# codename0og/codename-rvc-fork-3

Hardware: AMD Instinct MI355X
Metric: 48 kHz audio samples/sec end-to-end VC (higher is better)
Workload: dtype f32 (vocoder ResBlock convs and upsamplers, HuBERT, RMVPE's U-Net convs: fp32 operands as exact bf16x3 splits on the bf16 matrix cores -- six products of order <= 2^-16 per multiply-add, fp32 accumulate; everything else fp32 / fp64)

## Files before the change

### codename-rvc-fork-3_amd/csrc/linbf.hip

```cpp
#include <stdlib.h>

#include <mutex>
#include <vector>

#include "conv.h"

namespace rvc {

struct LinBfParams {
    const void *a = nullptr;
    const void *xs = nullptr;
    const float *bias = nullptr;
    float *y = nullptr;
    void *ys = nullptr;
    int M = 0, K = 0;
    int64_t N = 0, n_pad = 0;
    int mode = 0;
    int64_t x_row_stride = 0, x_plane = 0;
    int steps_per_part = 0;
    int n_col_blocks = 0;
};

constexpr int LBF_BN = 128, LBF_NTH = 512;
constexpr int LBF_SLAB_STEP = 12 * 1024;
constexpr int LBF_B_CHUNK = 3 * LBF_BN * 64;
typedef void __attribute__((address_space(3))) *lbf_lptr_t;

template <int MI>
struct LbfGeom {
    static constexpr int BM = 64 * MI;
    static constexpr int A_STEP = 2 * MI * 3 * 1024;
    static constexpr int D = MI == 2 ? 2 : 1;
    static constexpr int A_RING = 2 * (D + 1), B_RING = D + 1;
    static constexpr int NPIECE = 2 * 2 * MI * 3 + 24;
    static constexpr int UPW = (NPIECE + 7) / 8;
    static constexpr int LDS_USED = A_RING * A_STEP + B_RING * LBF_B_CHUNK;
    static_assert(LDS_USED <= 163840, "");
};

template <int MI>
__global__ void __launch_bounds__(LBF_NTH) __attribute__((amdgpu_waves_per_eu(2, 2)))
linbf_kernel(const LinBfParams p) {
    using GM = LbfGeom<MI>;
    constexpr int BM = GM::BM, A_STEP = GM::A_STEP, D = GM::D, A_RING = GM::A_RING, B_RING = GM::B_RING, NPIECE = GM::NPIECE, UPW = GM::UPW;
    extern __shared__ __attribute__((aligned(16))) unsigned char lbf_smem[];
    unsigned char *const a_ring = lbf_smem;
    unsigned char *const b_ring = lbf_smem + A_RING * A_STEP;
    const int tid = threadIdx.x, lane = tid & 63;
    const int wave = __builtin_amdgcn_readfirstlane(tid >> 6);
    __builtin_assume(wave >= 0 && wave < 8);
    const int wm = wave >> 2, wn = wave & 3;
    const int half = lane >> 5, l31 = lane & 31;
    const int n_m = p.M / BM;
    const int xcd = blockIdx.x & 7, slot = blockIdx.x >> 3;
// ... 98 lines not shown
                    if (p.bias) o += *reinterpret_cast<const f32x4 *>(p.bias + mb + 4 * half + 8 * (2 * rp + g));
#pragma unroll
                    for (int r = 0; r < 4; ++r) o[r] = 0.5f * o[r] * (1.f + erff(o[r] * 0.70710678118654752f));
                    v[g][0] = f32x2{o[0], o[1]};
                    v[g][1] = f32x2{o[2], o[3]};
                }
#pragma unroll
                for (int sp = 0; sp < 3; ++sp) {
                    unsigned w[2][2];
#pragma unroll
                    for (int g = 0; g < 2; ++g)
#pragma unroll
                        for (int h = 0; h < 2; ++h) {
                            w[g][h] = split_word(v[g][h]);
                            v[g][h] = split_rest(v[g][h], w[g][h]);
                        }
                    const unsigned s0 = half ? w[0][0] : w[1][0], s1 = half ? w[0][1] : w[1][1];
                    const unsigned r0 = (unsigned)__shfl_xor((int)s0, 32, 64), r1 = (unsigned)__shfl_xor((int)s1, 32, 64);
                    const u32x4 out = half ? u32x4{r0, r1, w[1][0], w[1][1]} : u32x4{w[0][0], w[0][1], r0, r1};
                    const int m = mb + 16 * rp + 8 * half;
                    if (live) *reinterpret_cast<u32x4 *>(reinterpret_cast<unsigned char *>(p.ys) + (((int64_t)sp * p.n_pad + n) * p.M + m) * 2) = out;
                }
            }
        }
        return;
    }
#pragma unroll
    for (int mi = 0; mi < MI; ++mi) {
        const int64_t n = n0 + nrow;
        if (n >= p.N) continue;
        const int mb = m0 + wm * 32 * MI + mi * 32 + 4 * half;
#pragma unroll
        for (int rg = 0; rg < 4; ++rg) {
            const int m = mb + 8 * rg;
            f32x4 o;
#pragma unroll
            for (int r = 0; r < 4; ++r) o[r] = acc[mi][4 * rg + r];
            if (p.mode == 2) {
                *reinterpret_cast<f32x4 *>(p.y + ((int64_t)part * p.N + n) * p.M + m) = o;
                continue;
            }
            if (p.bias) o += *reinterpret_cast<const f32x4 *>(p.bias + m);
            if (p.mode == 0) {
                *reinterpret_cast<f32x4 *>(p.y + n * p.M + m) = o;
                continue;
            }
#pragma unroll
            for (int r = 0; r < 4; ++r) o[r] = 0.5f * o[r] * (1.f + erff(o[r] * 0.70710678118654752f));
            *reinterpret_cast<f32x4 *>(p.y + n * p.M + m) = o;
        }
    }
}

__global__ void __launch_bounds__(256) split_rows_kernel(const float *__restrict__ x, unsigned char *__restrict__ xs, int64_t n_rows,
                                                          int64_t n_pad, int k) {
    const int64_t i4 = (int64_t)blockIdx.x * 256 + threadIdx.x;
    const int64_t total4 = n_rows * k / 4;
    if (i4 >= total4) return;
    const f32x4 v = *reinterpret_cast<const f32x4 *>(x + i4 * 4);
    f32x2 v0 = {v.x, v.y}, v1 = {v.z, v.w};
#pragma unroll
    for (int sp = 0; sp < 3; ++sp) {
        const unsigned w0 = split_word(v0), w1 = split_word(v1);
        *reinterpret_cast<u32x2 *>(xs + ((int64_t)sp * n_pad * k + i4 * 4) * 2) = u32x2{w0, w1};
        v0 = split_rest(v0, w0);
        v1 = split_rest(v1, w1);
    }
}

__device__ __forceinline__ float ln_row_mean(float sum, float inv_m) {
    float mean = sum * inv_m;
    asm volatile("" : "+v"(mean));
    return mean;
}

template <int PER_LANE>
__global__ void __launch_bounds__(256) ln_reduce_kernel(const float *__restrict__ parts, int n_parts, const float *__restrict__ bias,
                                                         const float *__restrict__ res, const float *__restrict__ gamma,
                                                         const float *__restrict__ beta, float eps, float *__restrict__ y,
                                                         unsigned char *__restrict__ ys, int64_t n_rows, int64_t n_pad) {
    constexpr int M = 64 * PER_LANE, Q = PER_LANE / 4;
    const int lane = threadIdx.x & 63;
    const int64_t n = (int64_t)blockIdx.x * 4 + (threadIdx.x >> 6);
    if (n >= n_rows) return;
    f32x4 v[Q];
#pragma unroll
    for (int q = 0; q < Q; ++q) {
        const int m = (q * 64 + lane) * 4;
        f32x4 a = bias ? *reinterpret_cast<const f32x4 *>(bias + m) : f32x4{0.f, 0.f, 0.f, 0.f};
        for (int s = 0; s < n_parts; ++s) a += *reinterpret_cast<const f32x4 *>(parts + ((int64_t)s * n_rows + n) * M + m);
        if (res) a += *reinterpret_cast<const f32x4 *>(res + n * M + m);
        v[q] = a;
    }
    float sum = 0.f;
#pragma unroll
    for (int q = 0; q < Q; ++q) sum += (v[q].x + v[q].y) + (v[q].z + v[q].w);
#pragma unroll
    for (int o = 32; o > 0; o >>= 1) sum += __shfl_xor(sum, o, 64);
    const float mean = ln_row_mean(sum, 1.f / M);
    float sq = 0.f;
#pragma unroll
    for (int q = 0; q < Q; ++q) {
        const f32x4 d = v[q] - mean;
        sq += (d.x * d.x + d.y * d.y) + (d.z * d.z + d.w * d.w);
    }
#pragma unroll
    for (int o = 32; o > 0; o >>= 1) sq += __shfl_xor(sq, o, 64);
    const float rstd = 1.f / sqrtf(sq * (1.f / M) + eps);
#pragma unroll
    for (int q = 0; q < Q; ++q) {
        const int m = (q * 64 + lane) * 4;
        f32x4 o = (v[q] - mean) * rstd;
        if (gamma) o *= *reinterpret_cast<const f32x4 *>(gamma + m);
        if (beta) o += *reinterpret_cast<const f32x4 *>(beta + m);
        if (y) *reinterpret_cast<f32x4 *>(y + n * M + m) = o;
        if (ys) {
            f32x2 v0 = {o.x, o.y}, v1 = {o.z, o.w};
#pragma unroll
            for (int sp = 0; sp < 3; ++sp) {
                const unsigned w0 = split_word(v0), w1 = split_word(v1);
                *reinterpret_cast<u32x2 *>(ys + (((int64_t)sp * n_pad + n) * M + m) * 2) = u32x2{w0, w1};
                v0 = split_rest(v0, w0);
                v1 = split_rest(v1, w1);
            }
        }
    }
}

template <int MI>
static int linbf_launch(LinBfParams p, int parts, hipStream_t stream) {
    if (reserve_whole_cu((const void *)linbf_kernel<MI>, "linear bf16x3 (pre-split)")) return 1;
    p.n_col_blocks = (int)ceil_div(p.N, LBF_BN);
    const int n_m = p.M / LbfGeom<MI>::BM;
    dim3 grid((unsigned)(ceil_div((int64_t)p.n_col_blocks * n_m, 8) * 8), (unsigned)parts, 1);
    hipLaunchKernelGGL(linbf_kernel<MI>, grid, dim3(LBF_NTH), LDS_WHOLE_CU, stream, p);
    RVC_LAUNCH_CHECK();
    return 0;
}

}

using namespace rvc;

extern "C" int rvc_split_rows_bf16x3(const float *x_dev, void *xs_dev, int64_t n_rows, int64_t n_rows_padded, int k, void *stream) {
    if (!x_dev || !xs_dev) return fail("rvc_split_rows_bf16x3: null pointer");
    if (k % 16 || n_rows_padded < n_rows || n_rows < 0) return fail("rvc_split_rows_bf16x3: k must be a multiple of 16, n_rows_padded >= n_rows");
    if (n_rows == 0) return 0;
    const int64_t total4 = n_rows * k / 4;
    hipLaunchKernelGGL(split_rows_kernel, dim3((unsigned)ceil_div(total4, 256)), dim3(256), 0, (hipStream_t)stream, x_dev,
                       reinterpret_cast<unsigned char *>(xs_dev), n_rows, n_rows_padded, k);
    RVC_LAUNCH_CHECK();
    return 0;
}

namespace {
int linbf_dispatch(const char *who, const void *xs_dev, int64_t x_row_stride, int64_t x_plane, const void *a_dev, const float *bias_dev,
                   float *y_dev, void *ys_dev, int64_t n_rows, int64_t n_rows_padded, int in_features, int out_features, int mode,
                   int k_parts, void *stream) {
    if (!xs_dev || !a_dev) return fail("%s: null pointer", who);
    if (out_features % 128 || in_features % 16) return fail("%s: out_features must be a multiple of 128, in_features of 16", who);
    if (mode < 0 || mode > 3) return fail("%s: mode must be 0 (fp32 + bias), 1 (bias + GELU -> planes), 2 (partial sums) or 3 (bias + GELU -> fp32)", who);
    if ((mode == 1) ? !ys_dev : !y_dev) return fail("%s: the output of mode %d is missing", who, mode);
    if (k_parts < 1 || (in_features / 32) % k_parts || in_features % 32) return fail("%s: in_features must be a multiple of 32 and k_parts divide in_features / 32", who);
    if (k_parts > 1 && mode != 2) return fail("%s: several K parts only produce partial sums (mode 2)", who);
    if (n_rows_padded % LBF_BN || n_rows_padded < n_rows) return fail("%s: n_rows_padded must be a multiple of 128 and >= n_rows", who);
    if (!fits_2gib((int64_t)out_features * in_features, 6) || !fits_2gib(3 * x_plane, 2) ||
        !fits_2gib((n_rows_padded + LBF_BN) * x_row_stride, 2))
        return fail("%s: an operand exceeds 2 GiB", who);
    if (x_row_stride % 8) return fail("%s: rows must start on 16-byte boundaries", who);
    if (n_rows <= 0) return 0;
    LinBfParams p;
    p.a = a_dev; p.xs = xs_dev; p.bias = bias_dev; p.y = y_dev; p.ys = ys_dev;
    p.M = out_features; p.K = in_features; p.N = n_rows; p.n_pad = n_rows_padded; p.mode = mode;
    p.x_row_stride = x_row_stride; p.x_plane = x_plane;
    p.steps_per_part = in_features / 16 / k_parts;
    const int64_t cols = ceil_div(n_rows, LBF_BN);
    const int cus = 256;
    auto cost = [&](int rows_per_block, double rel) {
        if (out_features % rows_per_block) return 1e30;
        return (double)ceil_div(cols * (out_features / rows_per_block) * k_parts, cus) * rel;
    };
    static const int by_cu_time = knob("RVC_LBF_TP", 0);
    if (by_cu_time) {
        auto cu_time = [&](int rows_per_block, double rel) { return out_features % rows_per_block ? 1e30 : cols * (out_features / rows_per_block) * k_parts * rel; };
        const double t128 = cu_time(128, 1.0), t192 = cu_time(192, 1.5 * 0.85), t256 = cu_time(256, 1.85);
        if (t192 <= t128 && t192 <= t256) return linbf_launch<3>(p, k_parts, (hipStream_t)stream);
        if (t256 < t128) return linbf_launch<4>(p, k_parts, (hipStream_t)stream);
        return linbf_launch<2>(p, k_parts, (hipStream_t)stream);
    }
    const double c128 = cost(128, 1.0), c192 = cost(192, 1.5 * 0.85), c256 = cost(256, 1.85);
    if (c256 < c128 && c256 <= c192) return linbf_launch<4>(p, k_parts, (hipStream_t)stream);
    const bool use192 = c192 < c128;
    return use192 ? linbf_launch<3>(p, k_parts, (hipStream_t)stream) : linbf_launch<2>(p, k_parts, (hipStream_t)stream);
}
}

extern "C" int rvc_linear_bf16x3_presplit(const void *xs_dev, const void *a_dev, const float *bias_dev, float *y_dev, void *ys_dev,
                                          int64_t n_rows, int64_t n_rows_padded, int in_features, int out_features, int mode, int k_parts,
                                          void *stream) {
    return linbf_dispatch("rvc_linear_bf16x3_presplit", xs_dev, in_features, n_rows_padded * in_features, a_dev, bias_dev, y_dev, ys_dev,
                          n_rows, n_rows_padded, in_features, out_features, mode, k_parts, stream);
}

extern "C" int rvc_conv1d_frames_bf16x3(const void *xs_dev, int64_t n_frames_in, int64_t n_frames_in_padded, int channels, int taps,
                                        int stride, const void *a_dev, const float *bias_dev, float *y_dev, void *ys_dev,
                                        int64_t n_frames_out_padded, int out_channels, int mode, void *stream) {
    if (taps < 1 || stride < 1 || channels < 8 || n_frames_in_padded < n_frames_in) return fail("rvc_conv1d_frames_bf16x3: bad argument");
    if (mode == 2) return fail("rvc_conv1d_frames_bf16x3: modes 0 (fp32 + bias), 1 (bias + GELU -> planes), 3 (bias + GELU -> fp32)");
    const int64_t n_out = n_frames_in >= taps ? (n_frames_in - taps) / stride + 1 : 0;
    return linbf_dispatch("rvc_conv1d_frames_bf16x3", xs_dev, (int64_t)stride * channels, n_frames_in_padded * channels, a_dev, bias_dev,
                          y_dev, ys_dev, n_out, n_frames_out_padded, taps * channels, out_channels, mode, 1, stream);
}

extern "C" int rvc_bias_residual_layernorm_bf16x3(const float *parts_dev, int n_parts, const float *bias_dev, const float *res_dev,
                                                  const float *gamma_dev, const float *beta_dev, float eps, float *y_dev, void *ys_dev,
                                                  int64_t n_rows, int64_t n_rows_padded, int features, void *stream) {
    if (!parts_dev || (!y_dev && !ys_dev)) return fail("rvc_bias_residual_layernorm_bf16x3: null pointer");
    if (n_parts < 1 || n_rows_padded < n_rows) return fail("rvc_bias_residual_layernorm_bf16x3: bad argument");
    if (n_rows <= 0) return 0;
    dim3 grid((unsigned)ceil_div(n_rows, 4));
    unsigned char *ys = reinterpret_cast<unsigned char *>(ys_dev);
    hipStream_t st = (hipStream_t)stream;
    if (features == 768)
        hipLaunchKernelGGL(ln_reduce_kernel<12>, grid, dim3(256), 0, st, parts_dev, n_parts, bias_dev, res_dev, gamma_dev, beta_dev, eps, y_dev, ys, n_rows, n_rows_padded);
    else if (features == 1024)
        hipLaunchKernelGGL(ln_reduce_kernel<16>, grid, dim3(256), 0, st, parts_dev, n_parts, bias_dev, res_dev, gamma_dev, beta_dev, eps, y_dev, ys, n_rows, n_rows_padded);
    else if (features == 256)
        hipLaunchKernelGGL(ln_reduce_kernel<4>, grid, dim3(256), 0, st, parts_dev, n_parts, bias_dev, res_dev, gamma_dev, beta_dev, eps, y_dev, ys, n_rows, n_rows_padded);
    else
        return fail("rvc_bias_residual_layernorm_bf16x3: features must be 256, 768 or 1024 (HuBERT-base: 768)");
    RVC_LAUNCH_CHECK();
    return 0;
}
```

### codename-rvc-fork-3_amd/rvc_amd/_native.py

```python
from __future__ import annotations

import ctypes
import threading
import os
from ctypes import POINTER, c_char_p, c_float, c_int, c_int64, c_size_t, c_void_p

import torch

_HERE = os.path.dirname(os.path.abspath(__file__))
LIB_PATH = os.path.join(_HERE, "_lib", "librvc_amd.so")
if os.environ.get("RVC_AMD_LIB"):
    LIB_PATH = os.path.abspath(os.environ["RVC_AMD_LIB"])
    print(f"[rvc_amd] RVC_AMD_LIB: loading {LIB_PATH} instead of the product library", flush=True)


class NativeError(RuntimeError):
    pass


if not os.path.isfile(LIB_PATH):
    raise ImportError(
        f"{LIB_PATH} is missing: build it with `python -c 'import __graft_entry__ as g; g.build()'` "
        "(hipcc --offload-arch=gfx950).  rvc_amd has no fallback path without its HIP library.")

# ... 62 lines not shown
    "rvc_decoder_set_tap": (c_int, [c_void_p, c_int, c_void_p]),
    "rvc_decoder_set_concurrency_hint": (c_int, [c_void_p, c_int]),
    "rvc_decoder_set_branch_parallel": (c_int, [c_void_p, c_int]),
    "rvc_posconv_bf16x3_weight_bytes": (c_int, [c_int, c_int, c_int, POINTER(c_size_t)]),
    "rvc_posconv_bf16x3_pack_weight": (c_int, [c_void_p, c_int, c_int, c_int, c_void_p, c_void_p]),
    "rvc_posconv_gelu_bf16x3": (c_int, [c_void_p, c_void_p, c_void_p, c_void_p, c_int64, c_int, c_int, c_int, c_int, c_void_p]),
    "rvc_hubert_conv0_workspace_bytes": (c_int, [c_int, POINTER(c_size_t)]),
    "rvc_hubert_conv0_frames_bf16x3": (c_int, [c_void_p, c_int64, c_void_p, c_int, c_int, c_int, c_void_p, c_void_p, c_float, c_void_p,
                                               c_size_t, c_void_p, c_int64, c_void_p]),
    "rvc_conv1d_frames_bf16x3": (c_int, [c_void_p, c_int64, c_int64, c_int, c_int, c_int, c_void_p, c_void_p, c_void_p, c_void_p, c_int64,
                                         c_int, c_int, c_void_p]),
    "rvc_conv1d_pack_weight": (c_int, [c_void_p, c_int, c_int, c_int, c_void_p, c_void_p]),
    "rvc_conv1d_forward": (c_int, [c_void_p, c_void_p, c_void_p, c_void_p, c_void_p, c_void_p, c_int, c_int, c_int,
                                   c_int64, c_int, c_int, c_float, c_float, c_void_p]),
    "rvc_conv1d_wino_pack_weight": (c_int, [c_void_p, c_int, c_int, c_int, c_void_p, c_void_p]),
    "rvc_conv1d_wino_forward": (c_int, [c_void_p, c_void_p, c_void_p, c_void_p, c_void_p, c_void_p, c_int, c_int, c_int,
                                        c_int64, c_int, c_int, c_float, c_float, c_void_p]),
    "rvc_conv1d_winobf_weight_bytes": (c_int, [c_int, c_int, c_int, POINTER(c_size_t)]),
    "rvc_conv1d_winobf_pack_weight": (c_int, [c_void_p, c_int, c_int, c_int, c_void_p, c_void_p]),
    "rvc_conv1d_winobf_forward": (c_int, [c_void_p, c_void_p, c_void_p, c_void_p, c_void_p, c_void_p, c_int, c_int, c_int,
                                          c_int64, c_int, c_int, c_float, c_float, c_void_p]),
    "rvc_resblock_bf16x3_weight_bytes": (c_int, [c_int, c_int, POINTER(c_size_t)]),
    "rvc_resblock_bf16x3_pack_weight": (c_int, [c_void_p, c_void_p, c_int, c_int, c_void_p, c_void_p]),
    "rvc_resblock_bf16x3_forward": (c_int, [c_void_p, c_void_p, c_void_p, c_void_p, c_void_p, c_void_p, c_int, c_int, c_int64, c_int,
                                            c_int, c_float, c_float, c_void_p]),
    "rvc_resblock_bf16w_weight_bytes": (c_int, [c_int, c_int, POINTER(c_size_t)]),
    "rvc_resblock_bf16w_pack_weight": (c_int, [c_void_p, c_void_p, c_int, c_int, c_void_p, c_void_p]),
    "rvc_resblock_bf16w_forward": (c_int, [c_void_p, c_void_p, c_void_p, c_void_p, c_void_p, c_void_p, c_int, c_int, c_int64, c_int,
                                           c_int, c_float, c_float, c_void_p]),
    "rvc_resblock_bf16x3_set_enabled": (c_int, [c_int]),
    "rvc_upsample_bf16x3_weight_bytes": (c_int, [c_int, c_int, c_int, c_int, c_int, c_int, POINTER(c_size_t)]),
    "rvc_upsample_bf16x3_pack_weight": (c_int, [c_void_p, c_void_p, c_void_p, c_int, c_int, c_int, c_int, c_int, c_int, c_void_p, c_void_p]),
    "rvc_upsample_bf16x3_forward": (c_int, [c_void_p, c_void_p, c_int64, c_void_p, c_void_p, c_void_p, c_int, c_int, c_int, c_int64, c_int, c_int,
                                            c_int, c_int, c_int, c_int, c_float, c_void_p]),
    "rvc_conv1d_f16x2_weight_bytes": (c_int, [c_int, c_int, POINTER(c_size_t)]),
    "rvc_conv1d_f16x2_pack_weight": (c_int, [c_void_p, c_int, c_int, c_void_p, c_void_p]),
    "rvc_conv1d_f16x2_forward": (c_int, [c_void_p, c_void_p, c_void_p, c_void_p, c_void_p, c_void_p, c_int, c_int, c_int64, c_int,
                                         c_int, c_float, c_float, c_void_p]),
    "rvc_decoder_set_arithmetic": (c_int, [c_void_p, c_int]),
    "rvc_conv1d_bf16w_weight_bytes": (c_int, [c_int, c_int, POINTER(c_size_t)]),
    "rvc_conv1d_bf16w_pack_weight": (c_int, [c_void_p, c_int, c_int, c_void_p, c_void_p]),
    "rvc_conv1d_bf16w_forward": (c_int, [c_void_p, c_void_p, c_void_p, c_void_p, c_void_p, c_void_p, c_int, c_int, c_int64, c_int,
                                         c_int, c_float, c_float, c_void_p]),
    "rvc_gemm_bf16x3_weight_bytes": (c_int, [c_int, c_int, POINTER(c_size_t)]),
    "rvc_gemm_bf16x3_pack_weight": (c_int, [c_void_p, c_int, c_int, c_int, c_void_p, c_void_p]),
    "rvc_linear_bf16x3": (c_int, [c_void_p, c_void_p, c_void_p, c_void_p, c_void_p, c_int64, c_int, c_int, c_int, c_void_p]),
    "rvc_conv1d_bf16x3": (c_int, [c_void_p, c_void_p, c_void_p, c_void_p, c_int, c_int, c_int, c_int64, c_int, c_int, c_int, c_int,
                                  c_void_p]),
    "rvc_split_rows_bf16x3": (c_int, [c_void_p, c_void_p, c_int64, c_int64, c_int, c_void_p]),
    "rvc_linear_bf16x3_presplit": (c_int, [c_void_p, c_void_p, c_void_p, c_void_p, c_void_p, c_int64, c_int64, c_int, c_int, c_int, c_int,
                                           c_void_p]),
    "rvc_bias_residual_layernorm_bf16x3": (c_int, [c_void_p, c_int, c_void_p, c_void_p, c_void_p, c_void_p, c_float, c_void_p, c_void_p,
                                                   c_int64, c_int64, c_int, c_void_p]),
    "rvc_conv2d_packed_floats": (c_int, [c_int, c_int, c_int, c_int, POINTER(c_size_t)]),
    "rvc_conv2d_pack_weight": (c_int, [c_void_p, c_int, c_int, c_int, c_int, c_void_p, c_void_p]),
    "rvc_conv2d_workspace_bytes": (c_int, [c_int, c_int, c_int, c_int, c_int, c_int, c_int, POINTER(c_size_t)]),
    "rvc_conv2d_bf16x3_supported": (c_int, [c_int, c_int, c_int, c_int]),
    "rvc_conv2d_bf16x3_weight_bytes": (c_int, [c_int, c_int, c_int, c_int, POINTER(c_size_t)]),
    "rvc_conv2d_bf16x3_pack_weight": (c_int, [c_void_p, c_int, c_int, c_int, c_int, c_void_p, c_void_p]),
    "rvc_conv2d_bf16x3_workspace_bytes": (c_int, [c_int, c_int, c_int, c_int, c_int, POINTER(c_size_t)]),
    "rvc_conv2d_bf16x3_forward": (c_int, [c_void_p, c_void_p, c_void_p, c_void_p, c_void_p, c_int, c_int, c_int, c_int, c_int, c_int,
                                          c_void_p, c_size_t, c_void_p]),
    "rvc_conv2d_forward": (c_int, [c_void_p, c_void_p, c_void_p, c_void_p, c_void_p, c_int, c_int, c_int, c_int, c_int, c_int,
                                   c_int, c_int, c_void_p, c_size_t, c_void_p]),
    "rvc_comm_unique_id": (c_int, [c_void_p]),
    "rvc_comm_create": (c_int, [c_void_p, c_int, c_int, POINTER(c_void_p)]),
    "rvc_comm_destroy": (c_int, [c_void_p]),
    "rvc_comm_info": (c_int, [c_void_p, POINTER(c_int), POINTER(c_int), POINTER(c_int), c_char_p, c_size_t]),
    "rvc_index_broadcast": (c_int, [c_void_p, c_void_p, c_size_t, c_int, c_void_p]),
    "rvc_checksum64": (c_int, [c_void_p, c_size_t, c_void_p, c_void_p]),
    "rvc_glu_dwconv_silu_f32": (c_int, [c_void_p, c_void_p, c_void_p, c_void_p, c_int64, c_int, c_int, c_void_p]),
    "rvc_layernorm_rows_f32": (c_int, [c_void_p, c_void_p, c_void_p, c_float, c_void_p, c_int64, c_int, c_void_p]),
    "rvc_groupnorm_workspace_bytes": (c_int, [c_int, c_int64, c_int, POINTER(c_size_t)]),
    "rvc_groupnorm_lrelu_f32": (c_int, [c_void_p, c_void_p, c_void_p, c_int, c_float, c_float, c_void_p, c_int, c_int64, c_void_p,
                                        c_size_t, c_void_p]),
    "rvc_fcpe_decode_f32": (c_int, [c_void_p, c_void_p, c_int, c_int, c_float, c_float, c_void_p, c_void_p, c_int64, c_void_p]),
    "rvc_kmeans_workspace_bytes": (c_int, [c_int64, c_int64, c_int, POINTER(c_size_t)]),
    "rvc_kmeans_assign": (c_int, [c_void_p, c_int64, c_int, c_void_p, c_int64, c_void_p, c_void_p, c_void_p, c_size_t, c_void_p]),
    "rvc_kmeans_update": (c_int, [c_void_p, c_int64, c_int, c_void_p, c_void_p, c_int64, c_void_p, c_void_p, c_void_p, c_size_t,
                                  c_void_p]),
    "rvc_lfilter_order5_warmup": (c_int, [c_void_p, POINTER(c_int64)]),
    "rvc_lfilter_order5_f64": (c_int, [c_void_p, c_int64, c_void_p, c_void_p, c_void_p]),
    "rvc_frame_rms_frames": (c_int, [c_int64, c_int64, c_int64, POINTER(c_int64), POINTER(c_size_t)]),
    "rvc_frame_rms_f64": (c_int, [c_void_p, c_int64, c_int64, c_int64, c_void_p, c_int64, c_void_p, c_size_t, c_void_p]),
    "rvc_slice_export_f32": (c_int, [c_void_p, c_int64, c_void_p, c_void_p, c_void_p, c_void_p, c_int64, c_int, c_int, c_void_p,
                                     c_int64, c_void_p, c_int64, c_void_p, c_int64, c_void_p]),
    "rvc_spectral_gate_params": (c_int, [c_int, POINTER(c_int), POINTER(c_int), POINTER(ctypes.c_double), c_void_p, c_void_p]),
    "rvc_spectral_gate_workspace_bytes": (c_int, [c_int64, c_int, c_int64, c_int64, POINTER(c_size_t)]),
    "rvc_spectral_gate_f32": (c_int, [c_void_p, c_int64, c_int, c_float, c_int64, c_int64, c_void_p, c_void_p, c_size_t, c_void_p]),
    "rvc_formant_shift_workspace_bytes": (c_int, [c_int64, c_int, POINTER(c_size_t)]),
    "rvc_formant_shift_f32": (c_int, [c_void_p, c_int64, c_int, ctypes.c_double, ctypes.c_double, c_int, c_void_p, c_void_p, c_size_t,
                                      c_void_p]),
}

for _name, (_res, _args) in SYMBOLS.items():
    _fn = getattr(_lib, _name)
    _fn.restype = _res
    _fn.argtypes = _args

ABI_VERSION = 4
if _lib.rvc_abi_version() != ABI_VERSION:
    raise ImportError(f"librvc_amd.so ABI {_lib.rvc_abi_version()} != {ABI_VERSION}: rebuild it")


def _check(rc: int, what: str):
    if rc != 0:
# ... 691 lines not shown
    ws = _workspace("groupnorm", x.device, "rvc_groupnorm_workspace_bytes", c, length, groups)
    y = torch.empty_like(x)
    gamma, beta = _dev_f32(gamma, "gamma"), _dev_f32(beta, "beta")
    _call("rvc_groupnorm_lrelu_f32", _device(x, gamma, beta), x.data_ptr(), gamma.data_ptr(), beta.data_ptr(), groups, float(eps),
          float(slope), y.data_ptr(), c, length, ws.data_ptr(), ws.numel())
    return y


def fcpe_decode(logits: torch.Tensor, cent_table: torch.Tensor, out_dims: int, threshold: float, f0_min: float,
                want_latent: bool = False):
    logits, cent_table = _dev_f32(logits, "logits"), _dev_f32(cent_table, "cent_table")
    n_rows, ld = logits.shape
    if cent_table.numel() != out_dims:
        raise NativeError(f"cent_table has {cent_table.numel()} entries, out_dims is {out_dims}")
    dev = _device(logits, cent_table)
    f0 = torch.empty(n_rows, dtype=torch.float32, device=dev)
    latent = torch.empty((n_rows, out_dims), dtype=torch.float32, device=dev) if want_latent else None
    _call("rvc_fcpe_decode_f32", dev, logits.data_ptr(), cent_table.data_ptr(), out_dims, ld, float(threshold), float(f0_min),
          f0.data_ptr(), _ptr(latent), n_rows)
    return f0, latent


def rows_padded(n_rows: int, tile: int = 128) -> int:
    return -(-n_rows // tile) * tile


def planes_empty(n_rows: int, features: int, device) -> torch.Tensor:
    return torch.empty((3, rows_padded(n_rows), features), dtype=torch.bfloat16, device=device)


def split_rows_bf16x3(x: torch.Tensor, out: torch.Tensor | None = None) -> torch.Tensor:
    x = _dev_f32(x, "x")
    n_rows, k = x.shape
    xs = out if out is not None else planes_empty(n_rows, k, x.device)
    _call("rvc_split_rows_bf16x3", _device(x, xs), x.data_ptr(), xs.data_ptr(), n_rows, xs.shape[1], k)
    return xs


def linear_bf16x3_presplit(xs: torch.Tensor, a_packed: torch.Tensor, bias, n_rows: int, out_features: int, mode: str = "f32",
                           k_parts: int = 1, out: torch.Tensor | None = None) -> torch.Tensor:
    _, n_pad, in_features = xs.shape
    m = {"f32": 0, "gelu_planes": 1, "parts": 2, "gelu_f32": 3}[mode]
    if m in (0, 3):
        y = out if out is not None else torch.empty((n_rows, out_features), dtype=torch.float32, device=xs.device)
    elif m == 1:
        y = out if out is not None else torch.empty((3, n_pad, out_features), dtype=torch.bfloat16, device=xs.device)
    else:
        y = out if out is not None else torch.empty((k_parts, n_rows, out_features), dtype=torch.float32, device=xs.device)
    _call("rvc_linear_bf16x3_presplit", _device(xs, a_packed, bias, y), xs.data_ptr(), a_packed.data_ptr(), _ptr(bias),
          y.data_ptr() if m != 1 else None, y.data_ptr() if m == 1 else None, n_rows, n_pad, in_features, out_features, m, k_parts)
    return y


def posconv_bf16x3_pack_weight(w: torch.Tensor, groups: int, device) -> torch.Tensor:
    w = _host(w)
    return _pack_slab("rvc_posconv_bf16x3", device, (w,), (w.shape[0], groups, w.shape[2]))


def posconv_gelu_bf16x3(x: torch.Tensor, a_packed: torch.Tensor, bias, groups: int, taps: int, padding: int) -> torch.Tensor:
    x = _dev_f32(x, "x")
    t, d = x.shape
    y = torch.empty_like(x)
    _call("rvc_posconv_gelu_bf16x3", _device(x, a_packed, bias), x.data_ptr(), a_packed.data_ptr(), _ptr(bias), y.data_ptr(), t, d, groups,
          taps, padding)
    return y


def hubert_conv0_frames_bf16x3(wav: torch.Tensor, w: torch.Tensor, gamma, beta, eps: float, stride: int = 5) -> tuple[torch.Tensor, int]:
    wav = _dev_f32(wav, "wav")
    w2 = _dev_f32(w.reshape(w.shape[0], -1), "w")
    dev = _device(wav, w2, gamma, beta)
    c, taps = w2.shape
    n = wav.numel()
    frames = (n - taps) // stride + 1
    ys = planes_empty(frames, c, dev)
    ws = _workspace("hubert_conv0", dev, "rvc_hubert_conv0_workspace_bytes", c)
    _call("rvc_hubert_conv0_frames_bf16x3", dev, wav.data_ptr(), n, w2.data_ptr(), c, taps, stride, _ptr(gamma), _ptr(beta), float(eps),
          ws.data_ptr(), ws.numel(), ys.data_ptr(), ys.shape[1])
    return ys, frames


def conv1d_frames_bf16x3(xs: torch.Tensor, n_frames_in: int, a_packed: torch.Tensor, bias, out_channels: int, taps: int, stride: int,
                         mode: str = "gelu_planes") -> tuple[torch.Tensor, int]:
    _, n_pad_in, c = xs.shape
    m = {"f32": 0, "gelu_planes": 1, "gelu_f32": 3}[mode]
    frames = (n_frames_in - taps) // stride + 1
    if frames <= 0:
        raise NativeError("conv1d_frames_bf16x3: the input is shorter than one window")
    y = planes_empty(frames, out_channels, xs.device) if m == 1 else torch.empty((frames, out_channels), dtype=torch.float32, device=xs.device)
    _call("rvc_conv1d_frames_bf16x3", _device(xs, a_packed, bias), xs.data_ptr(), n_frames_in, n_pad_in, c, taps, stride, a_packed.data_ptr(),
          _ptr(bias), y.data_ptr() if m != 1 else None, y.data_ptr() if m == 1 else None, rows_padded(frames), out_channels, m)
    return y, frames


def bias_residual_layernorm_bf16x3(parts: torch.Tensor, bias, res, gamma, beta, eps: float, want_planes: bool = True,
                                   y: torch.Tensor | None = None, ys: torch.Tensor | None = None):
    n_parts, n_rows, m = parts.shape
    y = y if y is not None else torch.empty((n_rows, m), dtype=torch.float32, device=parts.device)
    if want_planes and ys is None:
        ys = planes_empty(n_rows, m, parts.device)
    _call("rvc_bias_residual_layernorm_bf16x3", _device(parts, bias, res, gamma, beta, y, ys), parts.data_ptr(), n_parts, _ptr(bias),
          _ptr(res), _ptr(gamma), _ptr(beta), float(eps), y.data_ptr(), _ptr(ys), n_rows, ys.shape[1] if ys is not None else n_rows, m)
    return y, ys


def conv1d_bf16x3(x: torch.Tensor, a_packed: torch.Tensor, bias, c_out: int, k: int, stride: int = 1, padding: int = 0,
# ... 166 lines not shown
```

### include/rvc_amd.h

```cpp
#ifndef RVC_AMD_H
#define RVC_AMD_H

#include <stddef.h>
#include <stdint.h>

#ifdef __cplusplus
extern "C" {
#endif

#define RVC_AMD_ABI_VERSION 4


int rvc_abi_version(void);
const char *rvc_last_error(void);


int rvc_knn_index_aux_bytes(int64_t n_rows, int dim, size_t *bytes);
int rvc_knn_index_build(const float *index_dev, int64_t n_rows, int dim, void *aux_dev, size_t aux_bytes, void *stream);

int rvc_knn_workspace_bytes(int64_t n_rows, int64_t n_queries, int dim, int k, size_t *bytes);

int rvc_knn_search(const float *index_dev, const void *aux_dev, int64_t n_rows, int dim,
                   const float *queries_dev, int64_t n_queries, int k,
                   float *out_d2_dev, int64_t *out_ids_dev,
// ... 136 lines not shown
int rvc_conv1d_wino_pack_weight(const float *w_host, int c_out, int c_in, int k, float *u_dev, void *stream);
int rvc_conv1d_wino_forward(const float *x_dev, const float *u_dev, const float *bias_dev, const float *res_dev,
                            const float *acc_dev, float *y_dev, int batch, int c_in, int c_out, int64_t length, int k,
                            int dilation, float slope_in, float out_scale, void *stream);

int rvc_conv1d_winobf_weight_bytes(int c_out, int c_in, int k, size_t *bytes);
int rvc_conv1d_winobf_pack_weight(const float *w_host, int c_out, int c_in, int k, void *u_dev, void *stream);
int rvc_conv1d_winobf_forward(const float *x_dev, const void *u_dev, const float *bias_dev, const float *res_dev,
                              const float *acc_dev, float *y_dev, int batch, int c_in, int c_out, int64_t length, int k,
                              int dilation, float slope_in, float out_scale, void *stream);

int rvc_resblock_bf16x3_weight_bytes(int c, int k, size_t *bytes);
int rvc_resblock_bf16x3_pack_weight(const float *w1_host, const float *w2_host, int c, int k, void *u_dev, void *stream);
int rvc_resblock_bf16x3_forward(const float *x_dev, const void *u_dev, const float *b1_dev, const float *b2_dev,
                                const float *acc_dev, float *y_dev, int batch, int c, int64_t length, int k, int dilation,
                                float slope, float out_scale, void *stream);
int rvc_resblock_bf16w_weight_bytes(int c, int k, size_t *bytes);
int rvc_resblock_bf16w_pack_weight(const float *w1_host, const float *w2_host, int c, int k, void *u_dev, void *stream);
int rvc_resblock_bf16w_forward(const float *x_dev, const void *u_dev, const float *b1_dev, const float *b2_dev,
                               const float *acc_dev, float *y_dev, int batch, int c, int64_t length, int k, int dilation,
                               float slope, float out_scale, void *stream);
int rvc_conv1d_bf16w_weight_bytes(int c, int k, size_t *bytes);
int rvc_conv1d_bf16w_pack_weight(const float *w_host, int c, int k, void *u_dev, void *stream);
int rvc_conv1d_bf16w_forward(const float *x_dev, const void *u_dev, const float *bias_dev, const float *res_dev,
                             const float *acc_dev, float *y_dev, int batch, int c, int64_t length, int k, int dilation,
                             float slope_in, float out_scale, void *stream);
int rvc_conv1d_f16x2_weight_bytes(int c, int k, size_t *bytes);
int rvc_conv1d_f16x2_pack_weight(const float *w_host, int c, int k, void *u_dev, void *stream);
int rvc_conv1d_f16x2_forward(const float *x_dev, const void *u_dev, const float *bias_dev, const float *res_dev,
                             const float *acc_dev, float *y_dev, int batch, int c, int64_t length, int k, int dilation,
                             float slope_in, float out_scale, void *stream);
int rvc_upsample_bf16x3_weight_bytes(int c_in, int c_out, int rate, int ksize, int nc_k, int nc_stride, size_t *bytes);
int rvc_upsample_bf16x3_pack_weight(const float *up_w_host, const float *noise_w_host, const float *bias_host, int c_in, int c_out,
                                    int rate, int ksize, int nc_k, int nc_stride, void *u_dev, void *stream);
int rvc_upsample_bf16x3_forward(const float *x_dev, const float *har_dev, int64_t har_len, const void *u_dev, const float *bias_dev,
                                float *y_dev, int batch, int c_in, int c_out, int64_t length_in, int rate, int ksize, int pad,
                                int nc_k, int nc_stride, int nc_pad, float slope_in, void *stream);
int rvc_resblock_bf16x3_set_enabled(int enabled);

int rvc_gemm_bf16x3_weight_bytes(int m, int k_total, size_t *bytes);
int rvc_gemm_bf16x3_pack_weight(const float *w_host, int m, int k_total, int conv_taps, void *a_dev, void *stream);
int rvc_linear_bf16x3(const float *x_dev, const void *a_dev, const float *bias_dev, const float *res_dev, float *y_dev,
                      int64_t n_rows, int in_features, int out_features, int act, void *stream);
int rvc_conv1d_bf16x3(const float *x_dev, const void *a_dev, const float *bias_dev, float *y_dev, int batch, int c_in,
                      int c_out, int64_t l_in, int k, int stride, int padding, int act, void *stream);

int rvc_split_rows_bf16x3(const float *x_dev, void *xs_dev, int64_t n_rows, int64_t n_rows_padded, int k, void *stream);
int rvc_linear_bf16x3_presplit(const void *xs_dev, const void *a_dev, const float *bias_dev, float *y_dev, void *ys_dev,
                               int64_t n_rows, int64_t n_rows_padded, int in_features, int out_features, int mode, int k_parts,
                               void *stream);
int rvc_bias_residual_layernorm_bf16x3(const float *parts_dev, int n_parts, const float *bias_dev, const float *res_dev,
                                       const float *gamma_dev, const float *beta_dev, float eps, float *y_dev, void *ys_dev,
                                       int64_t n_rows, int64_t n_rows_padded, int features, void *stream);

int rvc_hubert_conv0_workspace_bytes(int channels, size_t *bytes);
int rvc_hubert_conv0_frames_bf16x3(const float *wav_dev, int64_t n_samples, const float *w_dev, int channels, int taps, int stride,
                                   const float *gamma_dev, const float *beta_dev, float eps, void *workspace_dev,
                                   size_t workspace_bytes, void *ys_dev, int64_t n_frames_padded, void *stream);
int rvc_conv1d_frames_bf16x3(const void *xs_dev, int64_t n_frames_in, int64_t n_frames_in_padded, int channels, int taps, int stride,
                             const void *a_dev, const float *bias_dev, float *y_dev, void *ys_dev, int64_t n_frames_out_padded,
                             int out_channels, int mode, void *stream);

int rvc_posconv_bf16x3_weight_bytes(int d, int groups, int taps, size_t *bytes);
int rvc_posconv_bf16x3_pack_weight(const float *w_host, int d, int groups, int taps, void *a_dev, void *stream);
int rvc_posconv_gelu_bf16x3(const float *x_dev, const void *a_dev, const float *bias_dev, float *y_dev, int64_t n_frames, int d,
                            int groups, int taps, int padding, void *stream);

int rvc_glu_dwconv_silu_f32(const float *x_dev, const float *w_dev, const float *bias_dev, float *y_dev, int64_t n_rows, int C, int K,
                            void *stream);
int rvc_layernorm_rows_f32(const float *x_dev, const float *gamma_dev, const float *beta_dev, float eps, float *y_dev, int64_t n_rows,
                           int F, void *stream);
int rvc_groupnorm_workspace_bytes(int C, int64_t L, int groups, size_t *bytes);
int rvc_groupnorm_lrelu_f32(const float *x_dev, const float *gamma_dev, const float *beta_dev, int groups, float eps, float slope,
                            float *y_dev, int C, int64_t L, void *workspace_dev, size_t workspace_bytes, void *stream);
int rvc_fcpe_decode_f32(const float *logits_dev, const float *cent_table_dev, int out_dims, int ld, float threshold, float f0_min,
                        float *f0_dev, float *latent_dev, int64_t n_rows, void *stream);

int rvc_kmeans_workspace_bytes(int64_t n_rows, int64_t n_centroids, int dim, size_t *bytes);
int rvc_kmeans_assign(const float *x_dev, int64_t n_rows, int dim, const float *centroids_dev, int64_t n_centroids,
                      int32_t *out_ids_dev, float *out_d2_dev, void *workspace_dev, size_t workspace_bytes, void *stream);
int rvc_kmeans_update(const float *x_dev, int64_t n_rows, int dim, const int32_t *order_dev, const int64_t *offsets_dev,
                      int64_t n_centroids, const float *old_centroids_dev, float *out_centroids_dev, void *workspace_dev,
                      size_t workspace_bytes, void *stream);

int rvc_lfilter_order5_warmup(const double *coef_host, int64_t *warm);
int rvc_lfilter_order5_f64(const double *x_dev, int64_t n, const double *coef_host, double *y_dev, void *stream);
int rvc_frame_rms_frames(int64_t n, int64_t frame_length, int64_t hop, int64_t *n_frames, size_t *workspace_bytes);
int rvc_frame_rms_f64(const double *x_dev, int64_t n, int64_t frame_length, int64_t hop, double *out_dev, int64_t n_frames,
                      void *workspace_dev, size_t workspace_bytes, void *stream);
int rvc_slice_export_f32(const double *x_dev, int64_t n, const int64_t *bounds_host, const int64_t *seg_dev,
                         const int64_t *off_full_dev, const int64_t *off_lo_dev, int64_t n_seg, int up, int down,
                         const double *h_dev, int64_t n_taps, float *full_dev, int64_t n_full, float *lo_dev, int64_t n_lo,
                         void *stream);

int rvc_spectral_gate_params(int sr, int *nf, int *nt, double *b, double *freq_taps, double *time_taps);
int rvc_spectral_gate_workspace_bytes(int64_t n, int sr, int64_t chunk_size, int64_t padding, size_t *bytes);
int rvc_spectral_gate_f32(const float *y_dev, int64_t n, int sr, float prop_decrease, int64_t chunk_size, int64_t padding,
                          float *out_dev, void *workspace_dev, size_t workspace_bytes, void *hip_stream);

int rvc_formant_shift_workspace_bytes(int64_t n, int group_frames, size_t *bytes);
int rvc_formant_shift_f32(const float *x_dev, int64_t n, int sr, double quefrency_s, double distortion, int group_frames,
                          float *out_dev, void *workspace_dev, size_t workspace_bytes, void *hip_stream);

#ifdef __cplusplus
}
#endif
// ... 2 lines not shown
```

Before: 58.33 million.

## Add warp-specialized persistent tile kernel for pre-split bf16x3 linear layers

Adds a persistent, XCD-aware tile kernel for the pre-split bf16x3 linear path. Four waves are dedicated producers that stream activation chunks into a double-buffered LDS ring and write the epilogue (bias, GELU, re-split). The other four waves run the MFMA loop with register-prefetched weight slabs. A cost model picks this form over the existing block kernel when its estimated CU rounds are lower. It also exposes a form override and query API. The aim is to overlap loads and epilogue with matrix-core work, at the price of a much more complex kernel and a heuristic dispatch.

```diff
diff --git a/codename-rvc-fork-3_amd/csrc/linbf.hip b/codename-rvc-fork-3_amd/csrc/linbf.hip
--- a/codename-rvc-fork-3_amd/csrc/linbf.hip
+++ b/codename-rvc-fork-3_amd/csrc/linbf.hip
@@ -1,5 +1,6 @@
 #include <stdlib.h>
 
+#include <atomic>
 #include <mutex>
 #include <vector>
 
@@ -204,6 +205,231 @@
     }
 }
 
+constexpr int LBT_BM = 256, LBT_BN = 64, LBT_CK = 64;
+constexpr int LBT_ROWB = 3 * LBT_CK * 2 + 16;
+constexpr int LBT_X_BYTES = LBT_BN * LBT_ROWB;
+constexpr int LBT_IO_ROWB = LBT_BM * 4 + 16;
+constexpr int LBT_IO_BYTES = LBT_BN * LBT_IO_ROWB;
+static_assert(2 * LBT_X_BYTES + LBT_IO_BYTES <= 163840, "LDS budget");
+static_assert((LBT_ROWB / 16) % 2 == 1, "row stride must be an odd multiple of 16 bytes");
+
+struct LinBtParams : LinBfParams {
+    int n_nt = 0, parts = 1;
+    int n_tasks = 0, per_xcd = 0;
+};
+
+template <int DBG>
+__global__ void __launch_bounds__(LBF_NTH) __attribute__((amdgpu_waves_per_eu(2, 2)))
+linbf_tile_kernel(const LinBtParams p) {
+    extern __shared__ __attribute__((aligned(16))) unsigned char lbt_smem[];
+    unsigned char *const xring = lbt_smem;
+    unsigned char *const io = lbt_smem + 2 * LBT_X_BYTES;
+    const int tid = threadIdx.x, lane = tid & 63;
+    const int wave = __builtin_amdgcn_readfirstlane(tid >> 6);
+    __builtin_assume(wave >= 0 && wave < 8);
+    const int half = lane >> 5, l31 = lane & 31;
+    unsigned long long *const stamps = (DBG & 64) ? reinterpret_cast<unsigned long long *>(p.ys) + ((size_t)blockIdx.x * 2 + (wave >= 4 ? 1 : 0)) * 64 : nullptr;
+    int n_stamp = 0;
+    auto stamp = [&]() __attribute__((always_inline)) {
+        if constexpr ((DBG & 64) != 0) {
+            if ((wave == 0 || wave == 4) && lane == 0 && n_stamp < 64) stamps[n_stamp] = __builtin_readcyclecounter();
+            ++n_stamp;
+        }
+    };
+
+    const int xcd = blockIdx.x & 7, slot = blockIdx.x >> 3, nslot = gridDim.x >> 3;
+    const int task_end = (xcd + 1) * p.per_xcd < p.n_tasks ? (xcd + 1) * p.per_xcd : p.n_tasks;
+    const int task0 = xcd * p.per_xcd + slot;
+    if (task0 >= task_end) return;
+    const int my_tasks = (task_end - task0 + nslot - 1) / nslot;
+    const int NCH = p.steps_per_part / 4;
+    const int n_q = my_tasks * NCH;
+    auto decode = [&](int t, int &ft, int &part, int &nt) __attribute__((always_inline)) {
+        const int tk = task0 + t * nslot, fp = tk / p.n_nt;
+        nt = tk - fp * p.n_nt;
+        ft = fp / p.parts;
+        part = fp - ft * p.parts;
+    };
+
+    if (wave >= 4) {
+        __builtin_amdgcn_s_setprio(1);
+        const int mw = wave - 4;
+        const __amdgpu_buffer_rsrc_t xrs = __builtin_amdgcn_make_buffer_rsrc((void *)p.xs, 0, (int)(3 * p.x_plane * 2), RSRC_RAW32);
+        const int plane_b = (int)(p.x_plane * 2), row_b = (int)(p.x_row_stride * 2);
+        const int seg = lane & 7, r8 = lane >> 3;
+        u32x4 xr[6];
+        int is_t = 0, is_c = 0;
+        auto x_issue = [&]() __attribute__((always_inline)) {
+            int ft, part, nt;
+            decode(is_t, ft, part, nt);
+            const int kb = (part * p.steps_per_part * 16 + is_c * LBT_CK) * 2;
+#pragma unroll
+            for (int i = 0; i < 6; ++i) {
+                const int j = 4 * i + mw, row = 8 * (j & 7) + r8;
+                xr[i] = __builtin_amdgcn_raw_buffer_load_b128(xrs, (nt * LBT_BN + row) * row_b + seg * 16, (j >> 3) * plane_b + kb, 0);
+            }
+            if (++is_c == NCH) { is_c = 0; ++is_t; }
+        };
+        auto x_write = [&](int q) __attribute__((always_inline)) {
+            unsigned char *const xb = xring + (q & 1) * LBT_X_BYTES;
+#pragma unroll
+            for (int i = 0; i < 6; ++i) {
+                const int j = 4 * i + mw, row = 8 * (j & 7) + r8;
+                *reinterpret_cast<u32x4 *>(xb + row * LBT_ROWB + (j >> 3) * (2 * LBT_CK) + seg * 16) = xr[i];
+            }
+        };
+        const int mode = p.mode;
+        auto gelu = [](float v) __attribute__((always_inline)) { return 0.5f * v * (1.f + erff(v * 0.70710678118654752f)); };
+        auto out_rows = [&](int t, int k0, int k1) __attribute__((always_inline)) {
+            int ft, part, nt;
+            decode(t, ft, part, nt);
+            const int m = ft * LBT_BM + 4 * lane;
+            f32x4 bv = {0.f, 0.f, 0.f, 0.f};
+            if (mode != 2 && p.bias) bv = *reinterpret_cast<const f32x4 *>(p.bias + m);
+#pragma unroll 1
+            for (int k = k0; k < k1; ++k) {
+                const int row = 4 * k + mw;
+                const int64_t n = (int64_t)nt * LBT_BN + row;
+                if (n >= p.N) continue;
+                const f32x4 v = *reinterpret_cast<const f32x4 *>(io + row * LBT_IO_ROWB + lane * 16);
+                if (mode == 2) {
+                    *reinterpret_cast<f32x4 *>(p.y + ((int64_t)part * p.N + n) * p.M + m) = v;
+                    continue;
+                }
+                float o[4] = {add_np(v.x, bv.x), add_np(v.y, bv.y), add_np(v.z, bv.z), add_np(v.w, bv.w)};
+                if (mode == 0) {
+                    *reinterpret_cast<f32x4 *>(p.y + n * p.M + m) = f32x4{o[0], o[1], o[2], o[3]};
+                    continue;
+                }
+#pragma unroll
+                for (int r = 0; r < 4; ++r) o[r] = gelu(o[r]);
+                if (mode == 3) {
+                    *reinterpret_cast<f32x4 *>(p.y + n * p.M + m) = f32x4{o[0], o[1], o[2], o[3]};
+                    continue;
+                }
+                unsigned w0[3], w1[3];
+                split3_np(o[0], o[1], w0);
+                split3_np(o[2], o[3], w1);
+#pragma unroll
+                for (int sp = 0; sp < 3; ++sp)
+                    *reinterpret_cast<u32x2 *>(reinterpret_cast<unsigned char *>(p.ys) + (((int64_t)sp * p.n_pad + n) * p.M + m) * 2) = u32x2{w0[sp], w1[sp]};
+            }
+        };
+        stamp();
+        x_issue();
+        x_write(0);
+        if (1 < n_q) x_issue();
+        int c = 0, t = 0;
+        for (int q = 0; q < n_q; ++q) {
+            lds_barrier();
+            stamp();
+            if (q + 1 < n_q) x_write(q + 1);
+            stamp();
+            asm volatile("s_waitcnt vmcnt(8)" ::: "memory");
+            if (q + 2 < n_q) x_issue();
+            stamp();
+            if (t > 0) out_rows(t - 1, 16 * c / NCH, 16 * (c + 1) / NCH);
+            stamp();
+            if (++c == NCH) {
+                c = 0;
+                ++t;
+                lds_barrier();
+            }
+        }
+        lds_barrier();
+        stamp();
+        out_rows(my_tasks - 1, 0, 16);
+        stamp();
+        return;
+    }
+
+    const __amdgpu_buffer_rsrc_t ars = __builtin_amdgcn_make_buffer_rsrc((void *)p.a, 0, (int)((int64_t)p.M * p.K * 6), RSRC_RAW32);
+    const int slab_row = (p.K / 16) * LBF_SLAB_STEP;
+    bf16x8 fa[4][6];
+    bf16x8 fb[2][2][3];
+    f32x16 acc[2][2];
+    auto base_of = [&](int t) __attribute__((always_inline)) {
+        int ft, part, nt;
+        decode(t, ft, part, nt);
+        return (2 * ft + (wave >> 1)) * slab_row + part * p.steps_per_part * LBF_SLAB_STEP + (wave & 1) * 6 * 1024;
+    };
+    int pf_t = 0, pf_s = 0, pf_base = base_of(0);
+    auto load_a1 = [&](int slot_a, int f) __attribute__((always_inline)) {
+        fa[slot_a][f] = __builtin_bit_cast(bf16x8, __builtin_amdgcn_raw_buffer_load_b128(ars, 16 * lane + f * 1024, pf_base + pf_s * LBF_SLAB_STEP, 0));
+    };
+    auto pf_next = [&]() __attribute__((always_inline)) {
+        if (++pf_s == p.steps_per_part) {
+            pf_s = 0;
+            ++pf_t;
+            pf_base = base_of(pf_t < my_tasks ? pf_t : my_tasks - 1);
+        }
+    };
+    auto load_b1 = [&](int buf, const unsigned char *src, int ks, int cb, int sp) __attribute__((always_inline)) {
+        fb[buf][cb][sp] = __builtin_bit_cast(bf16x8, *reinterpret_cast<const u32x4 *>(src + cb * 32 * LBT_ROWB + sp * (2 * LBT_CK) + ks * 32));
+    };
+#pragma unroll
+    for (int g = 0; g < 3; ++g) {
+#pragma unroll
+        for (int f = 0; f < 6; ++f) load_a1(g, f);
+        pf_next();
+    }
+    stamp();
+    const int x_lane = l31 * LBT_ROWB + half * 16;
+    unsigned char *const io_mine = io + l31 * LBT_IO_ROWB + (64 * wave + 4 * half) * 4;
+    constexpr int ia[6] = {2, 0, 1, 1, 0, 0}, ib[6] = {0, 2, 1, 0, 1, 0};
+    constexpr int po[3] = {0, 2, 1};
+
+    int q = 0;
+    for (int t = 0; t < my_tasks; ++t) {
+#pragma unroll
+        for (int mi = 0; mi < 2; ++mi)
+#pragma unroll
+            for (int cb = 0; cb < 2; ++cb)
+#pragma unroll
+                for (int r = 0; r < 16; ++r) acc[mi][cb][r] = 0.f;
+#pragma unroll 1
+        for (int c = 0; c < NCH; ++c, ++q) {
+            lds_barrier();
+            stamp();
+            const unsigned char *const src = xring + (q & 1) * LBT_X_BYTES + x_lane;
+#pragma unroll
+            for (int k = 0; k < 6; ++k) load_b1(0, src, 0, k & 1, po[k >> 1]);
+#pragma unroll
+            for (int ks = 0; ks < 4; ++ks) {
+#pragma unroll
+                for (int i = 0; i < 6; ++i)
+#pragma unroll
+                    for (int cb = 0; cb < 2; ++cb)
+#pragma unroll
+                        for (int mi = 0; mi < 2; ++mi) {
+                            const int k = (2 * i + cb) * 2 + mi;
+                            acc[mi][cb] = __builtin_amdgcn_mfma_f32_32x32x16_bf16(fa[ks][3 * mi + ia[i]], fb[ks & 1][cb][ib[i]], acc[mi][cb], 0, 0, 0);
+                            __builtin_amdgcn_sched_barrier(0);
+                            if (k < 6 && ks + 1 < 4) load_b1((ks + 1) & 1, src, ks + 1, k & 1, po[k >> 1]);
+                            if (k >= 18) {
+                                load_a1((ks + 3) & 3, k - 18);
+                                if (k == 23) pf_next();
+                            }
+                            __builtin_amdgcn_sched_barrier(0);
+                        }
+            }
+            stamp();
+        }
+        lds_barrier();
+        stamp();
+#pragma unroll
+        for (int mi = 0; mi < 2; ++mi)
+#pragma unroll
+            for (int cb = 0; cb < 2; ++cb)
+#pragma unroll
+                for (int rg = 0; rg < 4; ++rg)
+                    *reinterpret_cast<f32x4 *>(io_mine + cb * 32 * LBT_IO_ROWB + (32 * mi + 8 * rg) * 4) =
+                        f32x4{acc[mi][cb][4 * rg], acc[mi][cb][4 * rg + 1], acc[mi][cb][4 * rg + 2], acc[mi][cb][4 * rg + 3]};
+        stamp();
+    }
+    lds_barrier();
+}
+
 __global__ void __launch_bounds__(256) split_rows_kernel(const float *__restrict__ x, unsigned char *__restrict__ xs, int64_t n_rows,
                                                           int64_t n_pad, int k) {
     const int64_t i4 = (int64_t)blockIdx.x * 256 + threadIdx.x;
@@ -288,6 +514,60 @@
     hipLaunchKernelGGL(linbf_kernel<MI>, grid, dim3(LBF_NTH), LDS_WHOLE_CU, stream, p);
     RVC_LAUNCH_CHECK();
     return 0;
+}
+
+static int linbf_tile_launch(const LinBfParams &base, int parts, hipStream_t stream) {
+    if (reserve_whole_cu((const void *)linbf_tile_kernel<0>, "linear bf16x3 (pre-split, tile form)")) return 1;
+    LinBtParams p;
+    static_cast<LinBfParams &>(p) = base;
+    p.n_nt = (int)ceil_div(p.N, LBT_BN);
+    p.parts = parts;
+    p.n_tasks = (p.M / LBT_BM) * parts * p.n_nt;
+    const PersistentGrid g = persistent_grid(p.n_tasks);
+    p.per_xcd = g.per_xcd;
+#ifdef RVC_ABLATE
+    if (knob("RVC_LBT_DEBUG", 0) == 64 && p.mode == 0 && p.ys) {
+        if (reserve_whole_cu((const void *)linbf_tile_kernel<64>, "linear bf16x3 (pre-split, tile form, stamps)")) return 1;
+        hipLaunchKernelGGL(linbf_tile_kernel<64>, dim3(g.blocks), dim3(LBF_NTH), LDS_WHOLE_CU, stream, p);
+        RVC_LAUNCH_CHECK();
+        return 0;
+    }
+#endif
+    hipLaunchKernelGGL(linbf_tile_kernel<0>, dim3(g.blocks), dim3(LBF_NTH), LDS_WHOLE_CU, stream, p);
+    RVC_LAUNCH_CHECK();
+    return 0;
+}
+
+static std::atomic<int> lbf_form_mode{0};
+
+static bool linbf_tile_defined(int64_t n_rows, int in_features, int out_features, int k_parts) {
+    return out_features >= LBT_BM && out_features % LBT_BM == 0 && in_features % k_parts == 0 && in_features / k_parts >= LBT_CK &&
+           (in_features / k_parts) % LBT_CK == 0 &&
+           ceil_div(n_rows, LBT_BN) * (out_features / LBT_BM) * k_parts < ((int64_t)1 << 28);
+}
+
+constexpr int LBF_CUS = 256;
+static double linbf_block_rounds(int64_t n_rows, int out_features, int k_parts, int rows_per_block, double rel) {
+    if (out_features % rows_per_block) return 1e30;
+    return (double)ceil_div(ceil_div(n_rows, LBF_BN) * (out_features / rows_per_block) * k_parts, LBF_CUS) * rel;
+}
+static int linbf_block_mi(int64_t n_rows, int out_features, int k_parts) {
+    const double c128 = linbf_block_rounds(n_rows, out_features, k_parts, 128, 1.0), c192 = linbf_block_rounds(n_rows, out_features, k_parts, 192, 1.5 * 0.85),
+                 c256 = linbf_block_rounds(n_rows, out_features, k_parts, 256, 1.85);
+    if (c256 < c128 && c256 <= c192) return 4;
+    return c192 < c128 ? 3 : 2;
+}
+
+constexpr int LBF_FORM_BLOCK = 0, LBF_FORM_TILE = 1;
+static int linbf_form(int64_t n_rows, int in_features, int out_features, int k_parts) {
+    if (!linbf_tile_defined(n_rows, in_features, out_features, k_parts)) return LBF_FORM_BLOCK;
+    const int mode = lbf_form_mode.load(std::memory_order_relaxed);
+    if (mode == 1) return LBF_FORM_BLOCK;
+    if (mode == 2) return LBF_FORM_TILE;
+    const int mi = linbf_block_mi(n_rows, out_features, k_parts);
+    const double block = linbf_block_rounds(n_rows, out_features, k_parts, 64 * mi, mi == 2 ? 1.0 : mi == 3 ? 1.275 : 1.63);
+    const double tile = (double)ceil_div(ceil_div(n_rows, LBT_BN) * (out_features / LBT_BM) * k_parts, LBF_CUS) * 0.85;
+    return tile < block ? LBF_FORM_TILE : LBF_FORM_BLOCK;
 }
 
 }
@@ -326,24 +606,19 @@
     p.M = out_features; p.K = in_features; p.N = n_rows; p.n_pad = n_rows_padded; p.mode = mode;
     p.x_row_stride = x_row_stride; p.x_plane = x_plane;
     p.steps_per_part = in_features / 16 / k_parts;
-    const int64_t cols = ceil_div(n_rows, LBF_BN);
-    const int cus = 256;
-    auto cost = [&](int rows_per_block, double rel) {
-        if (out_features % rows_per_block) return 1e30;
-        return (double)ceil_div(cols * (out_features / rows_per_block) * k_parts, cus) * rel;
-    };
+    if (linbf_form(n_rows, in_features, out_features, k_parts) == LBF_FORM_TILE) return linbf_tile_launch(p, k_parts, (hipStream_t)stream);
     static const int by_cu_time = knob("RVC_LBF_TP", 0);
     if (by_cu_time) {
+        const int64_t cols = ceil_div(n_rows, LBF_BN);
         auto cu_time = [&](int rows_per_block, double rel) { return out_features % rows_per_block ? 1e30 : cols * (out_features / rows_per_block) * k_parts * rel; };
         const double t128 = cu_time(128, 1.0), t192 = cu_time(192, 1.5 * 0.85), t256 = cu_time(256, 1.85);
         if (t192 <= t128 && t192 <= t256) return linbf_launch<3>(p, k_parts, (hipStream_t)stream);
         if (t256 < t128) return linbf_launch<4>(p, k_parts, (hipStream_t)stream);
         return linbf_launch<2>(p, k_parts, (hipStream_t)stream);
     }
-    const double c128 = cost(128, 1.0), c192 = cost(192, 1.5 * 0.85), c256 = cost(256, 1.85);
-    if (c256 < c128 && c256 <= c192) return linbf_launch<4>(p, k_parts, (hipStream_t)stream);
-    const bool use192 = c192 < c128;
-    return use192 ? linbf_launch<3>(p, k_parts, (hipStream_t)stream) : linbf_launch<2>(p, k_parts, (hipStream_t)stream);
+    const int mi = linbf_block_mi(n_rows, out_features, k_parts);
+    if (mi == 4) return linbf_launch<4>(p, k_parts, (hipStream_t)stream);
+    return mi == 3 ? linbf_launch<3>(p, k_parts, (hipStream_t)stream) : linbf_launch<2>(p, k_parts, (hipStream_t)stream);
 }
 }
 
@@ -352,6 +627,25 @@
                                           void *stream) {
     return linbf_dispatch("rvc_linear_bf16x3_presplit", xs_dev, in_features, n_rows_padded * in_features, a_dev, bias_dev, y_dev, ys_dev,
                           n_rows, n_rows_padded, in_features, out_features, mode, k_parts, stream);
+}
+
+extern "C" int rvc_linear_bf16x3_form(int64_t n_rows, int in_features, int out_features, int k_parts) {
+    const char *who = "rvc_linear_bf16x3_form";
+    if (out_features <= 0 || in_features <= 0 || out_features % 128 || in_features % 16) {
+        fail("%s: out_features must be a multiple of 128, in_features of 16", who);
+        return -1;
+    }
+    if (k_parts < 1 || (in_features / 32) % k_parts || in_features % 32) {
+        fail("%s: in_features must be a multiple of 32 and k_parts divide in_features / 32", who);
+        return -1;
+    }
+    return n_rows > 0 ? linbf_form(n_rows, in_features, out_features, k_parts) : LBF_FORM_BLOCK;
+}
+
+extern "C" int rvc_linear_bf16x3_set_form(int mode) {
+    if (mode < 0 || mode > 2) return fail("rvc_linear_bf16x3_set_form: mode must be 0 (as measured), 1 (linbf_kernel) or 2 (the tile form wherever it is defined)");
+    lbf_form_mode.store(mode, std::memory_order_relaxed);
+    return 0;
 }
 
 extern "C" int rvc_conv1d_frames_bf16x3(const void *xs_dev, int64_t n_frames_in, int64_t n_frames_in_padded, int channels, int taps,
diff --git a/codename-rvc-fork-3_amd/rvc_amd/_native.py b/codename-rvc-fork-3_amd/rvc_amd/_native.py
--- a/codename-rvc-fork-3_amd/rvc_amd/_native.py
+++ b/codename-rvc-fork-3_amd/rvc_amd/_native.py
@@ -138,6 +138,8 @@
                                            c_void_p]),
     "rvc_bias_residual_layernorm_bf16x3": (c_int, [c_void_p, c_int, c_void_p, c_void_p, c_void_p, c_void_p, c_float, c_void_p, c_void_p,
                                                    c_int64, c_int64, c_int, c_void_p]),
+    "rvc_linear_bf16x3_form": (c_int, [c_int64, c_int, c_int, c_int]),
+    "rvc_linear_bf16x3_set_form": (c_int, [c_int]),
     "rvc_conv2d_packed_floats": (c_int, [c_int, c_int, c_int, c_int, POINTER(c_size_t)]),
     "rvc_conv2d_pack_weight": (c_int, [c_void_p, c_int, c_int, c_int, c_int, c_void_p, c_void_p]),
     "rvc_conv2d_workspace_bytes": (c_int, [c_int, c_int, c_int, c_int, c_int, c_int, c_int, POINTER(c_size_t)]),
@@ -935,6 +937,17 @@
     return y
 
 
+def linear_bf16x3_form(n_rows: int, in_features: int, out_features: int, k_parts: int = 1) -> int:
+    form = _lib.rvc_linear_bf16x3_form(n_rows, in_features, out_features, k_parts)
+    if form < 0:
+        raise NativeError(f"rvc_linear_bf16x3_form: {_lib.rvc_last_error().decode(errors='replace')}")
+    return form
+
+
+def linear_bf16x3_set_form(mode: int) -> None:
+    _check(_lib.rvc_linear_bf16x3_set_form(mode), "rvc_linear_bf16x3_set_form")
+
+
 def posconv_bf16x3_pack_weight(w: torch.Tensor, groups: int, device) -> torch.Tensor:
     w = _host(w)
     return _pack_slab("rvc_posconv_bf16x3", device, (w,), (w.shape[0], groups, w.shape[2]))
diff --git a/include/rvc_amd.h b/include/rvc_amd.h
--- a/include/rvc_amd.h
+++ b/include/rvc_amd.h
@@ -212,6 +212,8 @@
 int rvc_bias_residual_layernorm_bf16x3(const float *parts_dev, int n_parts, const float *bias_dev, const float *res_dev,
                                        const float *gamma_dev, const float *beta_dev, float eps, float *y_dev, void *ys_dev,
                                        int64_t n_rows, int64_t n_rows_padded, int features, void *stream);
+int rvc_linear_bf16x3_form(int64_t n_rows, int in_features, int out_features, int k_parts);
+int rvc_linear_bf16x3_set_form(int mode);
 
 int rvc_hubert_conv0_workspace_bytes(int channels, size_t *bytes);
 int rvc_hubert_conv0_frames_bf16x3(const float *wav_dev, int64_t n_samples, const float *w_dev, int channels, int taps, int stride,
```

Result: no change. 57.94 million (-0.7%).
